# donglinb/ORB-SLAM-BIRDVIEW

Measured on AMD Instinct MI355X. Metric: ORB features/sec per GPU (1280×720, 2000 kp, 8 levels) + Hamming matches/sec, higher is better.
Workload: dtype u8; 1 GPU; C3 1280x720 KITTI-style synthetic, 2000 features, 8 levels; width=1280, height=720, nfeatures=2000, nlevels=8, ini_th_fast=20, min_th_fast=7, batch_per_gpu=256, global_batch=256, parallelism=frame-sharded x1 (no collective), batches_in_flight=2

## Files before the change

orb-slam-birdview_amd/csrc/extract_kernels.hip:

```cpp
#include "glibc_trig.h"
#include "orbgpu_internal.h"
#include "pattern31_data.inc"

#include <algorithm>
#include <cstring>

namespace orbgpu {

__constant__ __attribute__((aligned(16))) int8_t c_pattern[1024] = {ORBGPU_PATTERN31_VALUES};
__constant__ __attribute__((aligned(16))) float c_pattern_f[1024] = {ORBGPU_PATTERN31_VALUES};

struct IcMaskTable {
    uint32_t m[64][4];
};
constexpr IcMaskTable make_ic_masks() {
    IcMaskTable t{};
    constexpr int umax[16] = {15, 15, 15, 15, 14, 14, 14, 13, 13, 12, 11, 10, 9, 8, 6, 3};
    for (int l = 0; l < 64; l++) {
        const int r = (l >> 1) < 30 ? (l >> 1) : 30, v = r - 15, h = l & 1;
        const int d = umax[v < 0 ? -v : v];
        for (int i = 0; i < 4; i++) {
            uint32_t m = 0;
            for (int j = 0; j < 4; j++) {
                const int u = 4 * (4 * h + i) + j;
// ... 786 lines not shown
    for (int j = 0; j < 4; j++) {
        const uint32_t P12 = __builtin_amdgcn_alignbyte(D[j + 1], D[j], 2);
        const uint32_t P4 = __builtin_amdgcn_alignbyte(D[j + 4], D[j + 3], 2);
        r[j] = compass2(D[j + 2], P[j], P4, M[j], P12, tt);
    }
    const uint32_t X = __builtin_amdgcn_perm(r[1], r[0], 0x07050301u);
    const uint32_t Y = __builtin_amdgcn_perm(r[3], r[2], 0x07050301u);
    const uint32_t Z = ((X >> 7) & 0x01010101u) | ((Y >> 3) & 0x10101010u);
    return __builtin_amdgcn_udot4(Z, 0x08040201u, 0u, false);
}

template <int TQ, bool TAIL>
__device__ __forceinline__ int prefilter_cell(const uint32_t* t32, int dh, int rpi, int lrow, bool lane_on, int lbase,
                                              uint32_t xvalid, uint32_t tt, uint16_t* sList, const FastCellT& c,
                                              const uint16_t* tile, int lane) {
    int nlist = 0;
    const int ntail = TAIL ? __builtin_amdgcn_readfirstlane(c.ntail) : 0;
    dh -= ntail;
    for (int r0 = 0; r0 < dh; r0 += rpi) {
        const int dy = r0 + lrow;
        int pm = 0;
        if (lane_on && dy < dh) {
            lds_cu32* w = (lds_cu32*)(t32 + r0 * (TQ / 2));
            asm volatile("" : "+v"(w));
            pm = (int)((prefilter16<TQ>(w, tt) | (prefilter16<TQ>(w + 4, tt) << 8)) & xvalid);
        }
        const int cnt = __popc(pm);
        const int incl = wave_incl_scan(cnt);
        int pos = nlist + incl - cnt;
        const int base = lbase + r0 * (2 * TQ);
        for (uint32_t b = (uint32_t)pm; b; b &= b - 1) sList[pos++] = (uint16_t)(base + 2 * __builtin_ctz(b));
        nlist += __builtin_amdgcn_readlane(incl, 63);
    }
    if (TAIL && ntail != 0) {
        const int np = __builtin_amdgcn_readfirstlane(c.np);
        const int trow = (int)div20(lane, c.m_np), pp = lane - trow * np;
        uint32_t r = 0;
        if (trow < ntail) {
            lds_cu32* q = (lds_cu32*)(reinterpret_cast<const uint32_t*>(tile) + ((dh + 3) * (TQ / 2) + 2)) +
                          (trow * (TQ / 2) + pp);
            const uint32_t l2 = q[-2], l1 = q[-1], v = q[0], r1 = q[1], r2 = q[2];
            const uint32_t P12 = __builtin_amdgcn_alignbyte(l1, l2, 2);
            const uint32_t P4 = __builtin_amdgcn_alignbyte(r2, r1, 2);
            r = compass2(v, q[3 * (TQ / 2)], P4, q[-3 * (TQ / 2)], P12, tt);
        }
        const bool lo = (r & 0x8000u) != 0, hi = (int)r < 0 && 2 * pp + 1 < c.dw;
        const unsigned long long ml = __ballot(lo), mh = __ballot(hi);
        const int pos = __builtin_amdgcn_mbcnt_hi((unsigned)(mh >> 32), __builtin_amdgcn_mbcnt_lo((unsigned)mh,
                        __builtin_amdgcn_mbcnt_hi((unsigned)(ml >> 32), __builtin_amdgcn_mbcnt_lo((unsigned)ml, nlist))));
        const int e = (dh + trow) * (2 * TQ) + 4 * pp;
        if (lo) sList[pos] = (uint16_t)e;
        if (hi) sList[pos + (lo ? 1 : 0)] = (uint16_t)(e + 2);
        nlist += __popcll(ml) + __popcll(mh);
    }
    return nlist;
}

template <int TQ, int CP = 0>
__device__ __forceinline__ void fast_cell_body(const Geom* __restrict__ g, const FastCellT& c, int lane,
                                               uint16_t* tile, uint16_t* sList,
                                               uint32_t* __restrict__ cands, uint32_t* __restrict__ candFirst,
                                               int* cntOut, unsigned long long* __restrict__ stamps, int item) {
    constexpr int PX = 16, TB = 2 * TQ;
    constexpr unsigned kRecipTB = (1u << 20) / TB + 1;
    const int dw = c.dw, dh = c.dh;
    ORBGPU_STAMP(1);
    const int nruns = c.nruns;
    const int rpi = c.rpi;
    const int lrow = (int)div20(lane, c.m_runs);
    const int x0 = PX * (lane - lrow * nruns);
    const bool lane_on = lrow < rpi;
    const uint32_t xvalid = x0 + PX <= dw ? (1u << PX) - 1u : (1u << max(dw - x0, 0)) - 1u;
    const int lpix = lrow * TQ + x0;
    const uint32_t* t32 = reinterpret_cast<const uint32_t*>(tile) + (lpix >> 1);
    uint8_t* t0 = reinterpret_cast<uint8_t*>(&tile[3 * TQ + 4]);
    int th = g->iniTh;
    int kept = 0;
    for (int pass = 0; pass < 2; pass++) {
        const uint32_t tt = (uint32_t)th | ((uint32_t)th << 16);
        const int nlist = prefilter_cell<TQ, (TQ < kFastTilePitch)>(t32, dh, rpi, lrow, lane_on, 2 * lpix, xvalid, tt,
                                                                    sList, c, tile, lane);
        wave_lds_sync();
        ORBGPU_STAMP(2);
#if defined(ORBGPU_FAST_CUT) && ORBGPU_FAST_CUT == 2
        if (lane == 0) *cntOut = nlist & 0;
        return;
#endif
        int ncorner = 0;
        for (int b0 = 0; b0 < nlist; b0 += 64) {
            const int i = b0 + lane;
            int p = 0, m = 0;
            if (i < nlist) {
                p = sList[i];
                m = fast_arc_strength<TB, 2>(t0 + p);
            }
            const bool corner = m > th;
            const unsigned long long cm = __ballot(corner);
            if (corner) {
                t0[p + 1] = (uint8_t)m;
                sList[ncorner + lanes_below(cm)] = (uint16_t)p;
            }
            ncorner += __popcll(cm);
        }
        wave_lds_sync();
        ORBGPU_STAMP(3);
#if defined(ORBGPU_FAST_CUT) && ORBGPU_FAST_CUT == 3
        if (lane == 0) *cntOut = ncorner & 0;
        return;
#endif
        kept = 0;
        for (int b0 = 0; b0 < ncorner; b0 += 64) {
            const int i = b0 + lane;
            bool k = false;
            uint32_t packed = 0;
            if (i < ncorner) {
                const int p = sList[i];
                const uint8_t* q = t0 + p + 1;
                const int m = q[0];
                const int s = m - 1;
                const int n0 = max(max((int)q[-TB - 2], (int)q[-TB]), (int)q[-TB + 2]);
                const int n1 = max(max((int)q[-2], (int)q[2]), 1);
                const int n2 = max(max((int)q[TB - 2], (int)q[TB]), (int)q[TB + 2]);
                k = m > max(max(n0, n1), n2);
                const int py = (int)(__umul24((unsigned)p, kRecipTB) >> 20), px = (p - py * TB) >> 1;
                packed = (uint32_t)(px + c.xo) | ((uint32_t)(py + c.yo) << 12) | ((uint32_t)s << 24);
            }
            const unsigned long long km = __ballot(k);
            const int slot = kept + lanes_below(km);
            if (k) {
                if constexpr (CP != 0) {
                    uint32_t* dst = slot < kCandFirst ? &candFirst[((long long)c.f * g->ncells + c.cell) * kCandRec + 1 + slot]
                                                      : &cands[(long long)c.f * g->ncand + c.out_off + slot];
                    __hip_atomic_store(dst, packed, __ATOMIC_RELAXED, __HIP_MEMORY_SCOPE_AGENT);
                } else {
                    if (slot < kCandFirst) candFirst[((long long)c.f * g->ncells + c.cell) * kCandRec + 1 + slot] = packed;
                    else cands[(long long)c.f * g->ncand + c.out_off + slot] = packed;
                }
            }
            kept += __popcll(km);
        }
        if (kept > 0 || th == g->minTh) break;
        th = g->minTh;
        for (int i = lane; i < ncorner; i += 64) t0[sList[i] + 1] = 0;
        wave_lds_sync();
    }
    ORBGPU_STAMP(4);
    if (lane == 0) {
        if constexpr (CP != 0) __hip_atomic_store(cntOut, kept, __ATOMIC_RELAXED, __HIP_MEMORY_SCOPE_AGENT);
        else *cntOut = kept;
    }
    ORBGPU_STAMP(5);
}

template <int TQ>
__global__ __launch_bounds__(256) void k_fast_wave(const Geom* __restrict__ g, const CellDesc* __restrict__ cells,
                                                   const uint8_t* __restrict__ frames,
                                                   long long framePitch, int rowStride, const uint8_t* __restrict__ pyr,
                                                   uint32_t* __restrict__ cands, uint32_t* __restrict__ candFirst,
                                                   int total,
                                                   int cbeg, int cnum, unsigned long long* __restrict__ stamps,
                                                   int* __restrict__ err, int ipw) {
    extern __shared__ __attribute__((aligned(16))) int smem_fast[];
    uint8_t* smem = reinterpret_cast<uint8_t*>(smem_fast);
    const int wv = __builtin_amdgcn_readfirstlane(threadIdx.x >> 6), lane = threadIdx.x & 63;
    const int nb = gridDim.x, q = nb >> 3, r = nb & 7, xcd = blockIdx.x & 7, j = blockIdx.x >> 3;
    const int blk = (xcd < r ? xcd * (q + 1) : r * (q + 1) + (xcd - r) * q) + j;
    const int item0 = (blk * (int)(blockDim.x >> 6) + wv) * ipw;
    if (item0 >= total) return;
    const int wb = g->fast_wave_bytes;
    uint16_t* tile = reinterpret_cast<uint16_t*>(smem + (size_t)wv * wb + 16);
    uint16_t* sList = reinterpret_cast<uint16_t*>(smem + (size_t)wv * wb + ((g->fast_rows * TQ * 2 + 32 + 15) & ~15));
    const bool has1 = ipw == 2 && item0 + 1 < total;
    const FastCellT c0 = fast_cell_t(g, cells, item0, frames, framePitch, rowStride, pyr, cbeg, cnum);
    const FastCellT c1 = fast_cell_t(g, cells, has1 ? item0 + 1 : item0, frames, framePitch, rowStride, pyr, cbeg, cnum);
    u32x2_t v0[8], v1[8];
    if (c0.valid && c0.aligned) fast_roi_issue(c0, lane, v0);
    if (has1 && c1.valid && c1.aligned) fast_roi_issue(c1, lane, v1);
    if (err && blockIdx.x == 0 && threadIdx.x == 0) {
        err[0] = 0;
        if (cnum == g->ncells) err[1] = 0;
    }
#pragma unroll
    for (int k = 0; k < 2; k++) {
        if (k == 1 && !has1) break;
        const FastCellT& c = k == 0 ? c0 : c1;
        const int item = item0 + k;
        int* cntOut = reinterpret_cast<int*>(candFirst + ((long long)c.f * g->ncells + c.cell) * kCandRec);
        if (!c.valid) {
            if (lane == 0) *cntOut = 0;
            continue;
        }
        ORBGPU_STAMP(0);
        wave_lds_sync();
        fast_roi_store<TQ>(c, lane, k == 0 ? v0 : v1, tile);
        ORBGPU_STAMP(6);
#if defined(ORBGPU_FAST_CUT) && ORBGPU_FAST_CUT == 1
        wave_lds_sync();
        if (lane == 0) *cntOut = (int)tile[lane] & 0;
        continue;
#endif
        fast_cell_body<TQ>(g, c, lane, tile, sList, cands, candFirst, cntOut, stamps, item);
    }
}

void fast_wave_layout(Geom& g) {
    int rows = 1, drows = 1, list = 1, maxw = 1;
    for (int l = 0; l < g.nlevels; l++) {
        const LevelGeom& L = g.L[l];
        rows = std::max(rows, L.hCell + 6);
        drows = std::max(drows, L.hCell);
        list = std::max(list, L.hCell * L.wCell);
        maxw = std::max(maxw, L.wCell);
    }
    g.fast_rows = rows;
    g.fast_drows = drows;
    g.fast_list = list;
    g.fast_compact = maxw <= 36 ? 1 : 0;
    const int tq = g.fast_compact ? 48 : kFastTilePitch;
    g.fast_wave_bytes = ((rows * tq * 2 + 32 + 15) & ~15) + ((list * 2 + 15) & ~15);
    g.fast_wave_bytes = (g.fast_wave_bytes + 15) & ~15;
}

__device__ __forceinline__ int quadrant_of(uint32_t key, uint32_t rx, uint32_t ry) {
    const int x = key & 0xFFF, y = (key >> 12) & 0xFFF;
    const int x0 = rx & 0xFFFF, x1 = rx >> 16, y0 = ry & 0xFFFF, y1 = ry >> 16;
    const int hx = (x1 - x0 + 1) >> 1, hy = (y1 - y0 + 1) >> 1;
    return (x >= x0 + hx ? 1 : 0) | (y >= y0 + hy ? 2 : 0);
}

__device__ __forceinline__ void child_rect(uint32_t rx, uint32_t ry, int q, uint32_t& crx, uint32_t& cry) {
    const int x0 = rx & 0xFFFF, x1 = rx >> 16, y0 = ry & 0xFFFF, y1 = ry >> 16;
    const int hx = (x1 - x0 + 1) >> 1, hy = (y1 - y0 + 1) >> 1;
    const int xm = x0 + hx, ym = y0 + hy;
    const int cx0 = (q & 1) ? xm : x0, cx1 = (q & 1) ? x1 : xm;
    const int cy0 = (q & 2) ? ym : y0, cy1 = (q & 2) ? y1 : ym;
    crx = (uint32_t)cx0 | ((uint32_t)cx1 << 16);
    cry = (uint32_t)cy0 | ((uint32_t)cy1 << 16);
}

template <int CP>
__device__ __forceinline__ int tidx() {
    if constexpr (CP == 0) return threadIdx.x;
    int t;
    asm volatile("v_mov_b32 %0, %1" : "=v"(t) : "v"((int)threadIdx.x));
    return t;
}

template <int NT, int CP = 0>
__device__ __forceinline__ int oct_scan(int v, int* sc, int& par, int& total) {
    constexpr int NW = NT / 64;
    const int lane = tidx<CP>() & 63, wave = tidx<CP>() >> 6;
    const int x = wave_incl_scan(v);
    int* buf = sc + 16 * par;
    par ^= 1;
    if (lane == 63) buf[wave] = x;
    __syncthreads();
    int pre = 0, tot = 0;
#pragma unroll
    for (int i = 0; i < NW; i++) {
        const int t = buf[i];
        pre += i < wave ? t : 0;
        tot += t;
    }
    total = tot;
    return pre + x - v;
}

template <int CP = 0>
__device__ __forceinline__ void wave_agg_add(int* ctr, bool ok, int tgt) {
    unsigned long long pending = __ballot(ok);
    while (pending) {
        const int leader = __ffsll((long long)pending) - 1;
        const int tl = __builtin_amdgcn_readlane(tgt, leader);
        const unsigned long long m = __ballot(ok && tgt == tl);
        if ((int)(tidx<CP>() & 63) == leader) atomicAdd(&ctr[tl], __popcll(m));
        pending &= ~m;
    }
}

__device__ __forceinline__ int quad_mask(const int* qd) {
    return (qd[0] > 0) | ((qd[1] > 0) << 1) | ((qd[2] > 0) << 2) | ((qd[3] > 0) << 3);
}

constexpr int kFfMaxDepth = 6;
constexpr int kFfPosShift = 20;
static_assert(kFfMaxNodes <= 1 << (32 - kFfPosShift), "a list position must fit above the count");

__device__ __forceinline__ int ff_depth(int nIni, int N, int room) {
    int F = 0, tot = 0, want = kFfMaxDepth;
    for (int d = 1; d <= kFfMaxDepth; d++)
        if ((nIni << (2 * d)) >= N) {
            want = d;
            break;
        }
    for (int d = 1; d <= want && d <= kFfMaxDepth; d++) {
        const int sz = nIni << (2 * d);
        if (sz > 65536 || tot + sz > room) break;
        tot += sz;
        F = d;
    }
    return F;
}

__device__ __forceinline__ int ff_base(int nIni, int d) { return nIni * (((1 << (2 * d)) - 4) / 3); }

template <int CP, class T>
__device__ __forceinline__ void oct_out(T* p, T v) {
    if constexpr (CP != 0) __hip_atomic_store(p, v, __ATOMIC_RELAXED, __HIP_MEMORY_SCOPE_AGENT);
    else *p = v;
}

template <bool KeysInLds, int NT, int CP = 0>
__device__ __forceinline__ void octree_level(const Geom* __restrict__ g, const LevelGeom& L, int f, int l, int* smem,
                                             int C, uint32_t* keys, uint16_t* knode, uint32_t* __restrict__ lvlKps,
                                             int* __restrict__ lvlCount, int* __restrict__ err, int par,
                                             unsigned long long* __restrict__ ost) {
    const int NC = g->node_cap;
    const int tid = tidx<CP>();
    const int tieMask = (g->variant & ORB_VARIANT_TIE_REVERSE) ? 0xFFFFFF : 0;
    uint32_t* rxA = (uint32_t*)smem;
    uint32_t* ryA = rxA + NC;
    int* cntA = (int*)(ryA + NC);
    int* seqA = cntA + NC;
    uint32_t* rxB = (uint32_t*)(seqA + NC);
    uint32_t* ryB = rxB + NC;
    int* cntB = (int*)(ryB + NC);
    int* seqB = cntB + NC;
    int* quad = seqB + NC;
    int* rank = quad + 4 * NC;
    int* info = rank + NC;
    int* ord = info + NC;
    int* nchr = ord + NC;
    int* sc = nchr + NC;
    int* sv = sc + 32;
#if ORBGPU_KERNEL_STAMPS
#define OCT_STAMP(k) \
    if (ost && tid == 0) ost[(k)] = __builtin_amdgcn_s_memtime();
#else
#define OCT_STAMP(k)
#endif

    __syncthreads();
    OCT_STAMP(1);
    if (ost && tid == 0) ost[29] = (unsigned long long)C;

    const int N = L.nfeat;
    const int nIni = L.nIni;
    const float hX = L.hX;
    const int Hn = L.maxBY - kMinBorder;
    if (nIni > NC) {
        if (tid == 0) { atomicOr(err, 1); oct_out<CP>(&lvlCount[f * g->nlevels + l], 0); }
        return;
    }
    int S = 0, nextSeq = 0, phase = 1, round0 = 0;
    bool ffDone = false, quadReady = false;
    const int F = C < (1 << 20) ? ff_depth(nIni, N, 8 * NC) : 0;
    if (F > 0) {
        int* T = quad;
        int* ffc = reinterpret_cast<int*>(rxB);
        const int bF = ff_base(nIni, F);
        const int szF = nIni << (2 * F);
        for (int t = tid; t < szF; t += NT) T[bF + t] = 0;
        for (int t = tid; t < 2 * (kFfMaxDepth + 1); t += NT) ffc[t] = 0;
        __syncthreads();
        OCT_STAMP(12);
        for (int i = tid; i < C; i += NT) {
            const uint32_t k = keys[i];
            const int x = k & 0xFFF, y = (k >> 12) & 0xFFF;
            const int t = min((int)((float)x / hX), nIni - 1);
            int x0 = (int)(hX * (float)t), x1 = (int)(hX * (float)(t + 1)), y0 = 0, y1 = Hn;
            int code = t;
            for (int d = 1; d <= F; d++) {
                const int xm = x0 + ((x1 - x0 + 1) >> 1), ym = y0 + ((y1 - y0 + 1) >> 1);
                const bool bx = x >= xm, by = y >= ym;
                x0 = bx ? xm : x0;
                x1 = bx ? x1 : xm;
                y0 = by ? ym : y0;
                y1 = by ? y1 : ym;
                code = code * 4 + ((int)bx | ((int)by << 1));
            }
            knode[i] = (uint16_t)code;
            atomicAdd(&T[bF + code], 1);
        }
        __syncthreads();
        OCT_STAMP(13);
        for (int d = F - 1; d >= 0; d--) {
            const int sz = d == 0 ? nIni : nIni << (2 * d);
            int* td = d == 0 ? cntB : T + ff_base(nIni, d);
            const int* tc = T + ff_base(nIni, d + 1);
            int dn = 0, en = 0, d0 = 0, e0 = 0;
            for (int c = tid; c < sz; c += NT) {
                const int4 ch = *reinterpret_cast<const int4*>(&tc[4 * c]);
                const int pc = ch.x + ch.y + ch.z + ch.w;
                td[c] = pc;
                if (pc >= 2) {
                    dn += (ch.x > 0) + (ch.y > 0) + (ch.z > 0) + (ch.w > 0);
                    en += (ch.x > 1) + (ch.y > 1) + (ch.z > 1) + (ch.w > 1);
                }
                d0 += pc > 0;
                e0 += pc > 1;
            }
            dn = wave_sum(dn);
            en = wave_sum(en);
            if ((tidx<CP>() & 63) == 0 && (dn | en)) {
                atomicAdd(&ffc[2 * (d + 1)], dn);
                atomicAdd(&ffc[2 * (d + 1) + 1], en);
            }
            if (d == 0) {
                d0 = wave_sum(d0);
                e0 = wave_sum(e0);
                if ((tidx<CP>() & 63) == 0 && (d0 | e0)) {
                    atomicAdd(&ffc[0], d0);
                    atomicAdd(&ffc[1], e0);
                }
            }
            __syncthreads();
        }
        OCT_STAMP(14);
        int Sr = ffc[0], Eprev = ffc[1], R = 0, base = 0, nseq = 0;
        bool fin = false, ph2 = false, over = false;
        for (int r = 1; r <= F; r++) {
            const int Dr = ffc[2 * r], Er = ffc[2 * r + 1];
            const int prev = Sr;
            Sr = Sr - Eprev + Dr;
            base = nseq;
            nseq += Dr;
            R = r;
            if (Sr > NC) { over = true; break; }
            if (Sr >= N || Sr == prev) { fin = true; break; }
            if (Sr + Er * 3 > N) { ph2 = true; break; }
            Eprev = Er;
        }
        if (over) {
            if (tid == 0) { atomicOr(err, 2); oct_out<CP>(&lvlCount[f * g->nlevels + l], 0); }
            return;
        }
        const int DR = ffc[2 * R];
        int V = 0;
        for (int d = R; d >= 0; d--) V += d == 0 ? nIni : nIni << (2 * d);
        OCT_STAMP(15);
        int run = 0;
        for (int v0 = 0; v0 < V; v0 += NT) {
            const int v = v0 + tid;
            int c = 0, n = 0, d = 0;
            bool on = false;
            int* td = cntB;
            if (v < V) {
                int off = 0;
                d = R;
                for (;;) {
                    const int sz = d == 0 ? nIni : nIni << (2 * d);
                    if (v < off + sz) break;
                    off += sz;
                    d--;
                }
                const int p = v - off;
                const int lowMask = (1 << (2 * d)) - 1;
                const int rt = p >> (2 * d);
                c = (((d & 1) ? nIni - 1 - rt : rt) << (2 * d)) | ((p & lowMask) ^ (0x33333333 & lowMask));
                td = d == 0 ? cntB : T + ff_base(nIni, d);
                n = td[c] & 0xFFFFF;
                const int* ptab = d == 1 ? cntB : T + ff_base(nIni, d > 1 ? d - 1 : 1);
                const bool node = n > 0 && (d == 0 || (ptab[c >> 2] & 0xFFFFF) >= 2);
                on = node && (d == R || n == 1);
            }
            int tot;
            const int pos = run + oct_scan<NT, CP>(on ? 1 : 0, sc, par, tot);
            if (on) {
                const int t = c >> (2 * d);
                int x0 = (int)(hX * (float)t), x1 = (int)(hX * (float)(t + 1)), y0 = 0, y1 = Hn;
                for (int k2 = d - 1; k2 >= 0; k2--) {
                    const int q = (c >> (2 * k2)) & 3;
                    const int xm = x0 + ((x1 - x0 + 1) >> 1), ym = y0 + ((y1 - y0 + 1) >> 1);
                    x0 = (q & 1) ? xm : x0;
                    x1 = (q & 1) ? x1 : xm;
                    y0 = (q & 2) ? ym : y0;
                    y1 = (q & 2) ? y1 : ym;
                }
                rxA[pos] = (uint32_t)x0 | ((uint32_t)x1 << 16);
                ryA[pos] = (uint32_t)y0 | ((uint32_t)y1 << 16);
                cntA[pos] = n;
                seqA[pos] = d == 0 ? -1 - t : d == R ? base + DR - 1 - pos : base;
                td[c] = (int)((uint32_t)n | ((uint32_t)pos << kFfPosShift));
                if (d == R) ryB[pos] = (uint32_t)c;
            }
            run += tot;
        }
        __syncthreads();
        OCT_STAMP(16);
        for (int i = tid; i < C; i += NT) {
            const int code = knode[i];
            int node = 0;
            for (int d = 0; d <= R; d++) {
                const int c = code >> (2 * (F - d));
                const int e = d == 0 ? cntB[c] : T[ff_base(nIni, d) + c];
                if (d == R || (e & 0xFFFFF) == 1) {
                    node = (int)((uint32_t)e >> kFfPosShift);
                    break;
                }
            }
            knode[i] = (uint16_t)node;
        }
        if (ph2 && R + 1 <= F) {
            constexpr int kMaxPer = 8;
            static_assert(kMaxPer * NT >= kFfMaxNodes, "every node of the list is read by some thread");
            int4 qv[kMaxPer];
            const int* tq = T + ff_base(nIni, R + 1);
#pragma unroll
            for (int j = 0; j < kMaxPer; j++) {
                const int pos = tid + j * NT;
                qv[j] = make_int4(0, 0, 0, 0);
                if (pos < run && pos < DR && cntA[pos] >= 2) qv[j] = *reinterpret_cast<const int4*>(&tq[4 * (int)ryB[pos]]);
            }
            __syncthreads();
#pragma unroll
            for (int j = 0; j < kMaxPer; j++) {
                const int pos = tid + j * NT;
                if (pos < run) *reinterpret_cast<int4*>(&quad[4 * pos]) = qv[j];
            }
            quadReady = true;
        }
        S = run;
        nextSeq = nseq;
        round0 = R;
        ffDone = fin;
        if (ph2) phase = 2;
    } else {
        for (int t = tid; t < nIni; t += NT) cntB[t] = 0;
        __syncthreads();
        for (int i0 = 0; i0 < C; i0 += NT) {
            const int i = i0 + tid;
            const bool ok = i < C;
            int r = 0;
            if (ok) {
                const int x = keys[i] & 0xFFF;
                r = min((int)((float)x / hX), nIni - 1);
                knode[i] = (uint16_t)r;
            }
            wave_agg_add<CP>(cntB, ok, r);
        }
        __syncthreads();
        for (int t0 = 0; t0 < nIni; t0 += NT) {
            const int t = t0 + tid;
            const int n = t < nIni ? cntB[t] : 0;
            int tot;
            const int pos = S + oct_scan<NT, CP>(n > 0 ? 1 : 0, sc, par, tot);
            if (n > 0) {
                const int x0 = (int)(hX * (float)t), x1 = (int)(hX * (float)(t + 1));
                rxA[pos] = (uint32_t)x0 | ((uint32_t)x1 << 16);
                ryA[pos] = (uint32_t)Hn << 16;
                cntA[pos] = n;
                seqA[pos] = -1 - t;
            }
            if (t < nIni) info[t] = pos;
            S += tot;
        }
        __syncthreads();
        for (int i = tid; i < C; i += NT) knode[i] = (uint16_t)info[knode[i]];
    }
    if (tid == 0) sv[3] = 0;
    __syncthreads();
    OCT_STAMP(2);

    for (int round = round0; round < 4 * NC + 64 && !ffDone; round++) {
        const int prevSize = S;
        [[maybe_unused]] const int subBase = round == 0 ? 12 : phase == 2 ? 20 : -1;
#if ORBGPU_KERNEL_STAMPS
#define OCT_SUB(k) \
    if (ost && tid == 0 && subBase >= 0 && subBase + (k) < 29) ost[subBase + (k)] = __builtin_amdgcn_s_memtime();
#else
#define OCT_SUB(k)
#endif
        if (!quadReady) for (int t = tid; t < 4 * S; t += NT) quad[t] = 0;
        for (int t = tid; t < S; t += NT) rank[t] = -1;
        __syncthreads();
        OCT_SUB(0);
        for (int i0 = 0; i0 < (quadReady ? 0 : C); i0 += 4 * NT) {
            int tt[4], tg[4];
            uint32_t kk[4];
            bool inc[4];
#pragma unroll
            for (int u = 0; u < 4; u++) {
                const int ic = min(i0 + u * NT + tid, C - 1);
                tt[u] = knode[ic];
                kk[u] = keys[ic];
            }
#pragma unroll
            for (int u = 0; u < 4; u++) {
                const int t = tt[u];
                inc[u] = i0 + u * NT + tid < C && cntA[t] > 1;
                tg[u] = 4 * t + quadrant_of(kk[u], rxA[t], ryA[t]);
            }
#pragma unroll
            for (int u = 0; u < 4; u++)
                if (inc[u]) atomicAdd(&quad[tg[u]], 1);
        }
        if (tid == 0) sv[4] = 0;
        __syncthreads();
        OCT_SUB(1);
        quadReady = false;
        int CH = 0, ndiv = 0;
        if (phase == 1) {
            int nproc = 0;
            for (int t0 = 0; t0 < S; t0 += NT) {
                const int t = t0 + tid;
                int val = 0, mask = 0;
                if (t < S && cntA[t] > 1) {
                    mask = quad_mask(&quad[4 * t]);
                    val = 1 | (__popc(mask) << 16);
                }
                int tot;
                const int pre = oct_scan<NT, CP>(val, sc, par, tot);
                if (t < S) {
                    if (val) {
                        rank[t] = nproc + (pre & 0xFFFF);
                        nchr[t] = CH + (pre >> 16);
                        info[t] = mask << 16;
                    } else {
                        info[t] = t - nproc - (pre & 0xFFFF);
                    }
                }
                nproc += tot & 0xFFFF;
                CH += tot >> 16;
            }
            ndiv = nproc;
            OCT_SUB(2);
        } else {
            int* dd = cntB;
            int* dpre = seqB;
            int nsort = 0;
            constexpr int kRkV = 32, NWv = NT / 64;
            const bool binned = 2 * NC >= kRkV * 16 && NC >= kRkV;
            if (binned) {
                int* T2 = reinterpret_cast<int*>(rxB);
                int* HV = seqB;
                int* ovl = nchr;
                const int lane = tid & 63, wave = tid >> 6;
                const bool rev = tieMask != 0;
                if (lane < kRkV) T2[lane * 16 + wave] = 0;
                const int PW = (S + NWv - 1) / NWv;
                const unsigned long long below = (1ull << lane) - 1ull;
                for (int c0 = wave * PW; c0 < min(S, (wave + 1) * PW); c0 += 64) {
                    const int pidx = c0 + lane;
                    const bool in = pidx < min(S, (wave + 1) * PW);
                    const int t = rev ? S - 1 - pidx : pidx;
                    const int cnt = in ? cntA[t] : 0;
                    const bool bg = cnt > 1;
                    const int v = min(cnt, kRkV - 1);
                    unsigned long long m = __ballot(bg);
#pragma unroll
                    for (int b = 0; b < 5; b++) {
                        const unsigned long long bal = __ballot((v >> b) & 1);
                        m &= ((v >> b) & 1) ? bal : ~bal;
                    }
                    const int prev = bg ? T2[v * 16 + wave] : 0;
                    __builtin_amdgcn_wave_barrier();
                    if (bg && (m & below) == 0) T2[v * 16 + wave] = prev + __popcll(m);
                    wave_lds_sync();
                    if (bg) {
                        info[t] = prev + __popcll(m & below);
                        if (v == kRkV - 1) ovl[atomicAdd(&sv[4], 1)] = t;
                    }
                }
                __syncthreads();
                for (int i = tid; i < kRkV * 16; i += NT) {
                    const int x = (i & 15) < NWv ? T2[i] : 0;
                    int y = x;
                    y += __builtin_amdgcn_update_dpp(0, y, 0x111, 0xf, 0xf, true);
                    y += __builtin_amdgcn_update_dpp(0, y, 0x112, 0xf, 0xf, true);
                    y += __builtin_amdgcn_update_dpp(0, y, 0x114, 0xf, 0xf, true);
                    y += __builtin_amdgcn_update_dpp(0, y, 0x118, 0xf, 0xf, true);
                    T2[i] = y - x;
                    if ((i & 15) == 15) HV[i >> 4] = y;
                }
                __syncthreads();
#pragma unroll 1
                for (int i = 0; i < kRkV; i += 4) {
                    const int4 h = *reinterpret_cast<const int4*>(&HV[i]);
                    nsort += h.x + h.y + h.z + h.w;
                }
                const int nov = sv[4];
                for (int t = tid; t < S; t += NT) {
                    const int cnt = cntA[t];
                    if (cnt <= 1) continue;
                    const int v = min(cnt, kRkV - 1);
                    const int pidx = rev ? S - 1 - t : t;
                    int r = 0;
                    if (v < kRkV - 1) {
                        r = info[t] + T2[v * 16 + pidx / PW];
#pragma unroll 1
                        for (int i = (v + 1) & ~3; i < kRkV; i += 4) {
                            const int4 h = *reinterpret_cast<const int4*>(&HV[i]);
                            r += (i > v ? h.x : 0) + (i + 1 > v ? h.y : 0) + (i + 2 > v ? h.z : 0) + (i + 3 > v ? h.w : 0);
                        }
                    } else {
                        for (int i = 0; i < nov; i++) {
                            const int u = ovl[i];
                            const int cu = cntA[u], pu = rev ? S - 1 - u : u;
                            r += cu > cnt || (cu == cnt && pu < pidx);
                        }
                    }
                    ord[r] = t;
                    dd[r] = __popc(quad_mask(&quad[4 * t])) - 1;
                }
                if (tid == 0) sv[2] = nsort;
                OCT_SUB(2);
            } else {
                unsigned long long* skey = reinterpret_cast<unsigned long long*>(rxB);
                for (int t0 = 0; t0 < S; t0 += NT) {
                    const int t = t0 + tid;
                    const bool big = t < S && cntA[t] > 1;
                    int tot;
                    const int pos = nsort + oct_scan<NT, CP>(big ? 1 : 0, sc, par, tot);
                    if (big)
                        skey[pos] = ((unsigned long long)cntA[t] << 40) |
                                    ((unsigned long long)((unsigned)(seqA[t] ^ tieMask) & 0xFFFFFFu) << 16) |
                                    (unsigned long long)t;
                    nsort += tot;
                }
                if (tid == 0) sv[2] = nsort;
                __syncthreads();
                OCT_SUB(2);
                const int G = nsort <= NT / 8 ? 8 : nsort <= NT / 4 ? 4 : nsort <= NT / 2 ? 2 : 1;
                const int lg = tid & (G - 1);
                for (int j0 = 0; j0 < nsort * G; j0 += NT) {
                    const int j = (j0 + tid) / G;
                    const bool ok = j < nsort;
                    const unsigned long long key = ok ? skey[j] : ~0ull;
                    int r = 0;
                    for (int i = 8 * lg; i + 8 <= nsort; i += 8 * G) {
                        const ulonglong2* p = reinterpret_cast<const ulonglong2*>(skey + i);
                        const ulonglong2 a = p[0], b = p[1], c = p[2], d = p[3];
                        r += (a.x > key) + (a.y > key) + (b.x > key) + (b.y > key) + (c.x > key) + (c.y > key) +
                             (d.x > key) + (d.y > key);
                    }
                    if (lg == 0)
                        for (int i = nsort & ~7; i < nsort; i++) r += skey[i] > key;
                    for (int o = 1; o < G; o <<= 1) r += __shfl_xor(r, o);
                    if (ok && lg == 0) {
                        const int t = (int)(key & 0xFFFF);
                        ord[r] = t;
                        dd[r] = __popc(quad_mask(&quad[4 * t])) - 1;
                    }
                }
            }
            __syncthreads();
            OCT_SUB(3);
            int run = 0;
            for (int r0 = 0; r0 < nsort; r0 += NT) {
                const int r = r0 + tid;
                const int d = r < nsort ? dd[r] : 0;
                int tot;
                const int pre = run + oct_scan<NT, CP>(d, sc, par, tot);
                if (r < nsort) dpre[r] = pre;
                const unsigned long long fail = __ballot(r < nsort && S + pre + d >= N);
                if (fail && (tidx<CP>() & 63) == 0) atomicMin(&sv[2], r0 + (tid & ~63) + __ffsll((long long)fail) - 1);
                run += tot;
            }
            __syncthreads();
            OCT_SUB(4);
            const int first_stop = sv[2];
            const int nproc = first_stop < nsort ? first_stop + 1 : nsort;
            ndiv = nproc;
            CH = nproc > 0 ? dpre[nproc - 1] + dd[nproc - 1] + nproc : 0;
            for (int r = tid; r < nproc; r += NT) {
                const int t = ord[r];
                rank[t] = r;
                nchr[t] = dpre[r] + r;
                info[t] = quad_mask(&quad[4 * t]) << 16;
            }
            __syncthreads();
            OCT_SUB(5);
            int und = 0;
            for (int t0 = 0; t0 < S; t0 += NT) {
                const int t = t0 + tid;
                const bool keep = t < S && rank[t] < 0;
                int tot;
                const int pre = und + oct_scan<NT, CP>(keep ? 1 : 0, sc, par, tot);
                if (keep) info[t] = pre;
                und += tot;
            }
            OCT_SUB(6);
        }
        const int Snew = CH + S - ndiv;
        if (Snew > NC) {
            if (tid == 0) { atomicOr(err, 2); oct_out<CP>(&lvlCount[f * g->nlevels + l], 0); }
            return;
        }
        int big = 0;
        for (int t0 = 0; t0 < S; t0 += NT) {
            const int t = t0 + tid;
            if (t >= S) break;
            const int rk = rank[t], inf = info[t], P = nchr[t], cnt = cntA[t], sq = seqA[t];
            const uint32_t rx = rxA[t], ry = ryA[t];
            const int4 qd = *reinterpret_cast<const int4*>(&quad[4 * t]);
            if (rk >= 0) {
                const int qc[4] = {qd.x, qd.y, qd.z, qd.w};
                const int mask = inf >> 16;
                const int start = CH - P - __popc(mask);
#pragma unroll
                for (int q = 0; q < 4; q++) {
                    if (!(mask & (1 << q))) continue;
                    const int pos = start + __popc(mask >> (q + 1));
                    uint32_t crx, cry;
                    child_rect(rx, ry, q, crx, cry);
                    rxB[pos] = crx;
                    ryB[pos] = cry;
                    cntB[pos] = qc[q];
                    seqB[pos] = nextSeq + P + __popc(mask & ((1 << q) - 1));
                    big += qc[q] > 1;
                }
                info[t] = start | (mask << 16);
            } else {
                const int pos = CH + inf;
                rxB[pos] = rx;
                ryB[pos] = ry;
                cntB[pos] = cnt;
                seqB[pos] = sq;
                info[t] = pos;
            }
        }
        big = wave_sum(big);
        if ((tidx<CP>() & 63) == 0 && big) atomicAdd(&sv[3], big);
        __syncthreads();
        OCT_SUB(phase == 1 ? 3 : 7);
        for (int i0 = 0; i0 < C; i0 += 4 * NT) {
            int tt[4], nt[4];
            uint32_t kk[4];
#pragma unroll
            for (int u = 0; u < 4; u++) {
                const int ic = min(i0 + u * NT + tid, C - 1);
                tt[u] = knode[ic];
                kk[u] = keys[ic];
            }
#pragma unroll
            for (int u = 0; u < 4; u++) {
                const int t = tt[u];
                const int inf = info[t], rk = rank[t];
                const int q = quadrant_of(kk[u], rxA[t], ryA[t]);
                nt[u] = rk >= 0 ? (inf & 0xFFFF) + __popc((inf >> 16) >> (q + 1)) : inf;
            }
#pragma unroll
            for (int u = 0; u < 4; u++)
                if (i0 + u * NT + tid < C) knode[i0 + u * NT + tid] = (uint16_t)nt[u];
        }
        const int nToExpand = sv[3];
        __syncthreads();
        OCT_SUB(phase == 1 ? 4 : 8);
        if (tid == 0) sv[3] = 0;
        {
            uint32_t* p = rxA; rxA = rxB; rxB = p;
            p = ryA; ryA = ryB; ryB = p;
            int* q = cntA; cntA = cntB; cntB = q;
            q = seqA; seqA = seqB; seqB = q;
        }
        nextSeq += CH;
        S = Snew;
        if (round < 9) OCT_STAMP(3 + round);
        if (S >= N || S == prevSize) break;
        if (phase == 1 && S + nToExpand * 3 > N) {
            phase = 2;
            if (ost && tid == 0) ost[30] = (unsigned long long)(round + 1);
        }
    }

#undef OCT_SUB
    uint32_t* best = (uint32_t*)quad;
    for (int t = tid; t < S; t += NT) best[t] = 0;
    __syncthreads();
    OCT_STAMP(17);
    for (int i = tid; i < C; i += NT) {
        const uint32_t v = ((keys[i] >> 24) << 24) | (uint32_t)(0xFFFFFF - i);
        atomicMax(&best[knode[i]], v);
    }
    __syncthreads();
    OCT_STAMP(18);
    uint32_t* outK = lvlKps + (long long)f * g->nkpcap + L.kp_base;
    for (int t = tid; t < S; t += NT) {
        const int i = 0xFFFFFF - (int)(best[t] & 0xFFFFFF);
        const uint32_t k = keys[i];
        const uint32_t x = (k & 0xFFF) + kMinBorder, y = ((k >> 12) & 0xFFF) + kMinBorder;
        oct_out<CP>(&outK[t], x | (y << 12) | (k & 0xFF000000u));
    }
    if (tid == 0) oct_out<CP>(&lvlCount[f * g->nlevels + l], S);
    OCT_STAMP(31);
#undef OCT_STAMP
}

template <int CP>
__device__ __forceinline__ uint32_t cand_slot(__amdgpu_buffer_rsrc_t rs, unsigned i) {
    return __builtin_amdgcn_raw_buffer_load_b32(rs, (int)(4 * i), 0, CP);
}

template <int NT, int CP>
__device__ __forceinline__ void octree_task(const Geom* __restrict__ g, int f, int l, int* smem,
                                            const uint32_t* __restrict__ cands, const uint32_t* __restrict__ candFirst,
                                            uint32_t* __restrict__ keysAll, uint16_t* __restrict__ knodeAll,
                                            uint32_t* __restrict__ lvlKps, int* __restrict__ lvlCount,
                                            int* __restrict__ err, int lds_keys, unsigned long long* __restrict__ ostamps) {
    const int NC = g->node_cap;
    const int tid = tidx<CP>();
    const LevelGeom& L = g->L[l];
    unsigned long long* ost = ostamps ? ostamps + ((long long)f * g->nlevels + l) * 32 : nullptr;
#if ORBGPU_KERNEL_STAMPS
    if (ost && tid == 0) ost[0] = __builtin_amdgcn_s_memtime();
#endif
    constexpr int kFirst = kCandFirst;
    const int ncl = L.nCols * L.nRows;
    const uint32_t* cs = cands + (long long)f * g->ncand + L.cand_base;
    const uint4* cf = reinterpret_cast<const uint4*>(candFirst) + ((long long)f * g->ncells + L.cell_base) * 2;
    const uint32_t* cr = candFirst + ((long long)f * g->ncells + L.cell_base) * kCandRec;
    static_assert(kCandRec == 8, "two uint4 per cell record");
    auto crsf = [&]() { return __builtin_amdgcn_make_buffer_rsrc(const_cast<uint32_t*>(cr), 0, ncl * kCandRec * 4, 0x00020000); };
    auto csrf = [&]() { return __builtin_amdgcn_make_buffer_rsrc(const_cast<uint32_t*>(cs), 0, L.cand_cap * 4, 0x00020000); };
    int* sc = smem + 16 * NC;
    int* sv = sc + 32;
    uint32_t* keysL = reinterpret_cast<uint32_t*>(sv + 8);
    const long long o = ((long long)f * g->nlevels + l) * g->max_level_cand;
    int par = 0;
    constexpr int kMaxChunks = 4;
    const int nch = (ncl + NT - 1) / NT;
    int C = 0;
    bool inLds;
    uint32_t* keys;
    if (nch <= kMaxChunks) {
        int n[kMaxChunks], off[kMaxChunks];
        uint32_t v[kMaxChunks][kFirst];
#pragma unroll
        for (int j = 0; j < kMaxChunks; j++) {
            n[j] = 0;
#pragma unroll
            for (int k = 0; k < kFirst; k++) v[j][k] = 0;
            const int c = j * NT + tid;
            if (j < nch && c < ncl) {
                uint4 r0, r1;
                if constexpr (CP != 0) {
                    const uint32x4_t a = __builtin_amdgcn_raw_buffer_load_b128(crsf(), 32 * c, 0, CP);
                    const uint32x4_t b = __builtin_amdgcn_raw_buffer_load_b128(crsf(), 32 * c + 16, 0, CP);
                    r0 = make_uint4(a[0], a[1], a[2], a[3]);
                    r1 = make_uint4(b[0], b[1], b[2], b[3]);
                } else {
                    r0 = cf[2 * c];
                    r1 = cf[2 * c + 1];
                }
                n[j] = (int)r0.x;
                v[j][0] = r0.y;
                v[j][1] = r0.z;
                v[j][2] = r0.w;
                v[j][3] = r1.x;
                v[j][4] = r1.y;
                v[j][5] = r1.z;
                v[j][6] = r1.w;
            }
        }
#pragma unroll
        for (int j = 0; j < kMaxChunks; j++) {
            if (j < nch) {
                int tot;
                off[j] = C + oct_scan<NT, CP>(n[j], sc, par, tot);
                C += tot;
            }
        }
        inLds = C <= lds_keys;
        keys = inLds ? keysL : keysAll + o;
#pragma unroll
        for (int j = 0; j < kMaxChunks; j++) {
            const int c = j * NT + tid;
            if (j < nch && c < ncl) {
#pragma unroll
                for (int k = 0; k < kFirst; k++)
                    if (k < n[j]) keys[off[j] + k] = v[j][k];
                if constexpr (CP != 0) {
                    for (int k = kFirst; k < n[j]; k++) keys[off[j] + k] = cand_slot<CP>(csrf(), __umul24((unsigned)c, (unsigned)L.cell_cap) + k);
                } else {
                    for (int k = kFirst; k < n[j]; k++) keys[off[j] + k] = cs[__umul24((unsigned)c, (unsigned)L.cell_cap) + k];
                }
            }
        }
    } else {
        int base = 0;
        for (int c0 = 0; c0 < ncl; c0 += NT) {
            const int c = c0 + tid;
            int n = 0;
            if constexpr (CP != 0) n = c < ncl ? (int)cand_slot<CP>(crsf(), (unsigned)c * kCandRec) : 0;
            else n = c < ncl ? (int)cr[(long long)c * kCandRec] : 0;
            int tot;
            (void)oct_scan<NT, CP>(n, sc, par, tot);
            base += tot;
        }
        C = base;
        inLds = C <= lds_keys;
        keys = inLds ? keysL : keysAll + o;
        base = 0;
        for (int c0 = 0; c0 < ncl; c0 += NT) {
            const int c = c0 + tid;
            int n = 0;
            if constexpr (CP != 0) n = c < ncl ? (int)cand_slot<CP>(crsf(), (unsigned)c * kCandRec) : 0;
            else n = c < ncl ? (int)cr[(long long)c * kCandRec] : 0;
            int tot;
            const int off = base + oct_scan<NT, CP>(n, sc, par, tot);
            if constexpr (CP != 0) {
                for (int k = 0; k < n; k++)
                    keys[off + k] = k < kFirst ? cand_slot<CP>(crsf(), (unsigned)c * kCandRec + 1 + k)
                                               : cand_slot<CP>(csrf(), __umul24((unsigned)c, (unsigned)L.cell_cap) + k);
            } else {
                for (int k = 0; k < n; k++)
                    keys[off + k] = k < kFirst ? cr[(long long)c * kCandRec + 1 + k]
                                               : cs[__umul24((unsigned)c, (unsigned)L.cell_cap) + k];
            }
            base += tot;
        }
    }
    if (inLds)
        octree_level<true, NT, CP>(g, L, f, l, smem, C, keys, reinterpret_cast<uint16_t*>(keysL + lds_keys), lvlKps, lvlCount,
                               err, par, ost);
    else
        octree_level<false, NT, CP>(g, L, f, l, smem, C, keys, knodeAll + o, lvlKps, lvlCount, err, par, ost);
}


template <int NT>
__global__ __launch_bounds__(NT) void k_octree(const Geom* __restrict__ g,
                                                           const uint32_t* __restrict__ cands,
                                                           const uint32_t* __restrict__ candFirst,
                                                           uint32_t* __restrict__ keysAll,
                                                           uint16_t* __restrict__ knodeAll,
                                                           uint32_t* __restrict__ lvlKps, int* __restrict__ lvlCount,
                                                           int* __restrict__ err, int lds_keys,
                                                           unsigned long long* __restrict__ ostamps, int lbase) {
    extern __shared__ __attribute__((aligned(16))) int smem[];
    octree_task<NT, 0>(g, blockIdx.x, lbase + (int)blockIdx.y, smem, cands, candFirst, keysAll, knodeAll, lvlKps,
                       lvlCount, err, lds_keys, ostamps);
}

constexpr float kAtanScale = (float)(180 / 3.14159265358979323846);
constexpr float kP1 = 0.9997878412794807f * kAtanScale;
constexpr float kP3 = -0.3258083974640975f * kAtanScale;
constexpr float kP5 = 0.1555786518463281f * kAtanScale;
constexpr float kP7 = -0.04432655554792128f * kAtanScale;
constexpr float kFactorPI = (float)(3.14159265358979323846 / 180.f);

__device__ __forceinline__ float fast_atan2(float y, float x) {
    const float ax = fabsf(x), ay = fabsf(y);
    float a, c, c2;
    if (ax >= ay) {
        c = ay / (ax + (float)2.220446049250313e-16);
        c2 = c * c;
        a = (((kP7 * c2 + kP5) * c2 + kP3) * c2 + kP1) * c;
    } else {
        c = ax / (ay + (float)2.220446049250313e-16);
        c2 = c * c;
        a = 90.f - (((kP7 * c2 + kP5) * c2 + kP3) * c2 + kP1) * c;
    }
    if (x < 0) a = 180.f - a;
    if (y < 0) a = 360.f - a;
    return a;
}



constexpr int kDescRtCols = 37, kDescWinOff = 2976, kDescWaveBytes = kDescWinOff + kDescWin * kDescWinPitch;
constexpr bool desc_overlap_ok() {
    return 2 * kRtPitch * kDescRtCols <= kDescWinOff + 6 * kDescWinPitch && kDescWinOff % 16 == 0 &&
           kDescWaveBytes % 16 == 0 && 4 * kDescWaveBytes + 256 <= 160 * 1024 / 8;
}
static_assert(desc_overlap_ok(), "k_describe LDS overlap");

struct DescSlot {
    bool ok, interior;
    int s, l, x, y, score, outIdx;
    LevelPtr src;
};

template <int CP = 0>
__device__ __forceinline__ DescSlot desc_slot(const Geom* __restrict__ g, int f, int s, const int* cnts,
                                              const uint32_t* __restrict__ lvlKps, const uint8_t* frames,
                                              long long framePitch, int rowStride, const uint8_t* pyr) {
    DescSlot d;
    d.s = s;
    d.ok = false;
    d.interior = false;
    if (s >= g->nkpcap) return d;
    const int nl = g->nlevels;
    int l = 0;
    while (l + 1 < nl && s >= g->L[l + 1].kp_base) ++l;
    const LevelGeom& L = g->L[l];
    const int k = s - L.kp_base;
    auto cnt = [&](int i) -> int {
        if constexpr (CP != 0) return __hip_atomic_load(&cnts[i], __ATOMIC_RELAXED, __HIP_MEMORY_SCOPE_AGENT);
        else return cnts[i];
    };
    if (k >= cnt(l)) return d;
    int outIdx = k;
    for (int i = 0; i < l; i++) outIdx += cnt(i);
    uint32_t kp;
    if constexpr (CP != 0) kp = __hip_atomic_load(&lvlKps[(long long)f * g->nkpcap + s], __ATOMIC_RELAXED, __HIP_MEMORY_SCOPE_AGENT);
    else kp = lvlKps[(long long)f * g->nkpcap + s];
    d.ok = true;
    d.l = l;
    d.x = kp & 0xFFF;
    d.y = (kp >> 12) & 0xFFF;
    d.score = kp >> 24;
    d.outIdx = outIdx;
    d.src = level_ptr(g, l, frames, framePitch, rowStride, pyr, f);
    const bool aligned = ((reinterpret_cast<uintptr_t>(d.src.p) | (uintptr_t)d.src.stride) & 3) == 0;
    d.interior = aligned && d.x >= 21 && d.x + 27 <= L.w && d.y >= 21 && d.y + 21 < L.h;
    return d;
}

template <int CP = 0>
__device__ __forceinline__ void desc_issue(const DescSlot& d, int lane, uint32_t (&v)[9]) {
    const int a0 = (d.x - 21) & ~3;
    const int stride = __builtin_amdgcn_readfirstlane(d.src.stride);
    const uint64_t rb = reinterpret_cast<uint64_t>(d.src.p + (long long)(d.y - 21) * stride + a0);
    const uint64_t rbu = ((uint64_t)(uint32_t)__builtin_amdgcn_readfirstlane((unsigned)(rb >> 32)) << 32) |
                         (uint64_t)(uint32_t)__builtin_amdgcn_readfirstlane((unsigned)rb);
    const auto rsrc = __builtin_amdgcn_make_buffer_rsrc(reinterpret_cast<void*>(rbu), 0, (kDescWin - 1) * stride + 48,
                                                          0x00020000);
    const int wy0 = (int)(__umul24((unsigned)lane, 2731u) >> 15), ww = lane - wy0 * 12;
    const int off = (int)roi_off(wy0, stride, 4 * ww);
#pragma unroll
    for (int r = 0; r < 8; r++) v[r] = __builtin_amdgcn_raw_buffer_load_b32(rsrc, off, 5 * r * stride, CP);
    v[8] = __builtin_amdgcn_raw_buffer_load_b32(rsrc, lane < 36 ? off : 0x40000000, 40 * stride, CP);
}

template <bool ALLEVEN, bool FMA>
__device__ __forceinline__ void brief_sampled(const uint16_t* rt, float a, float b, const float (&pf)[4][4], int colBase,
                                              int xsimd, ushort2_t K01, ushort2_t K23, ushort2_t K45, ushort2_t K60,
                                              int lane, unsigned long long* __restrict__ dst) {
    typedef const uint32_t __attribute__((address_space(3))) lds_u32;
    constexpr uint32_t kC = (uint32_t)kRtPitch * 0x400000u + 0x4B400000u;
    static_assert((kC & 1u) == 0, "the element bias must keep the parity");
    const uint32_t lbase = (uint32_t)(uintptr_t)(lds_u32*)reinterpret_cast<const uint32_t*>(rt) - 2u * kC;
    const uint32_t xlim = (uint32_t)(xsimd - colBase) + 0x4B400000u;
    const uint32_t bias = sgpr_const(32767u);
    typedef float f32x2_t __attribute__((ext_vector_type(2)));
    const f32x2_t ab = {a, b}, nba = {-b, a}, cr = {12582930.0f, 12582930.0f};
    auto sample = [&](f32x2_t pp) -> uint32_t {
        const f32x2_t pyv = __builtin_shufflevector(pp, pp, 1, 1), pxv = __builtin_shufflevector(pp, pp, 0, 0);
        const f32x2_t t = pyv * nba;
        const f32x2_t r = (FMA ? __builtin_elementwise_fma(pxv, ab, t) : pxv * ab + t) + cr;
        const float fx = r.x, fy = r.y;
        const uint32_t xbits = __builtin_bit_cast(uint32_t, fx);
        const uint32_t ybits = __builtin_bit_cast(uint32_t, fy);
        const uint32_t idx = __umul24(xbits, (unsigned)kRtPitch) + ybits;
        uint32_t ie = idx & ~1u;
        asm("" : "+v"(ie));
        lds_u32* rp = (lds_u32*)(uintptr_t)(lbase + (ie << 1));
        const uint32_t sh = idx << 4;
        const uint32_t d0 = rp[0], d1 = rp[1], d2 = rp[2], d3 = rp[3];
        uint32_t S = __builtin_amdgcn_udot2(K01, __builtin_bit_cast(ushort2_t, __builtin_amdgcn_alignbit(d1, d0, sh)), 0u, false);
        S = __builtin_amdgcn_udot2(K23, __builtin_bit_cast(ushort2_t, __builtin_amdgcn_alignbit(d2, d1, sh)), S, false);
        S = __builtin_amdgcn_udot2(K45, __builtin_bit_cast(ushort2_t, __builtin_amdgcn_alignbit(d3, d2, sh)), S, false);
        S = __builtin_amdgcn_udot2(K60, __builtin_bit_cast(ushort2_t, __builtin_amdgcn_alignbit(d3, d3, sh)), S, false);
        if (ALLEVEN) return S + bias + ((S >> 16) & 1u);
        return S + (xbits < xlim ? bias + ((S >> 16) & 1u) : 32768u);
    };
    unsigned long long mq[4];
#pragma unroll
    for (int gq = 0; gq < 4; gq++) {
        const uint32_t r0 = sample(f32x2_t{pf[gq][0], pf[gq][1]});
        const uint32_t r1 = sample(f32x2_t{pf[gq][2], pf[gq][3]});
        mq[gq] = __ballot((r0 >> 16) < min(r1 >> 16, 255u));
    }
    if (lane < 4) dst[lane] = lane == 0 ? mq[0] : lane == 1 ? mq[1] : lane == 2 ? mq[2] : mq[3];
}

// ... 890 lines not shown
```

Baseline: 410.4 million features/s.

## Drive phase-2 octree rounds from precomputed fast-forward count tables

Builds the fast-forward quadtree count table one level deeper and, when phase 2 begins within that depth, represents nodes as packed (depth, code) pairs. Child counts are then read directly from the table instead of rebucketing every keypoint each round. Keypoint-to-node assignment is deferred to a single lookup pass at the end, or runs when the tree grows past the tabled depth, at which point rectangles are reconstructed. The goal is to remove the per-round passes over all keypoints in the octree distribution. In exchange it uses more shared-memory table space, adds extra code paths, and adds a final fixup pass.

```diff
diff --git a/orb-slam-birdview_amd/csrc/extract_kernels.hip b/orb-slam-birdview_amd/csrc/extract_kernels.hip
--- a/orb-slam-birdview_amd/csrc/extract_kernels.hip
+++ b/orb-slam-birdview_amd/csrc/extract_kernels.hip
@@ -1112,7 +1112,28 @@
     return F;
 }
 
+__device__ __forceinline__ uint32_t ff_pack(int d, int c) { return ((uint32_t)d << 16) | (uint32_t)c; }
+
+__device__ __forceinline__ void ff_rect(float hX, int Hn, int d, int c, uint32_t& rx, uint32_t& ry) {
+    const int t = c >> (2 * d);
+    int x0 = (int)(hX * (float)t), x1 = (int)(hX * (float)(t + 1)), y0 = 0, y1 = Hn;
+    for (int k2 = d - 1; k2 >= 0; k2--) {
+        const int q = (c >> (2 * k2)) & 3;
+        const int xm = x0 + ((x1 - x0 + 1) >> 1), ym = y0 + ((y1 - y0 + 1) >> 1);
+        x0 = (q & 1) ? xm : x0;
+        x1 = (q & 1) ? x1 : xm;
+        y0 = (q & 2) ? ym : y0;
+        y1 = (q & 2) ? y1 : ym;
+    }
+    rx = (uint32_t)x0 | ((uint32_t)x1 << 16);
+    ry = (uint32_t)y0 | ((uint32_t)y1 << 16);
+}
+
 __device__ __forceinline__ int ff_base(int nIni, int d) { return nIni * (((1 << (2 * d)) - 4) / 3); }
+
+__device__ __forceinline__ int ff_table_depth(int nIni, int F, int keep) {
+    return F > 0 && (nIni << (2 * (F + 1))) <= 65536 && ff_base(nIni, F + 2) <= keep ? F + 1 : F;
+}
 
 template <int CP, class T>
 __device__ __forceinline__ void oct_out(T* p, T v) {
@@ -1164,14 +1185,17 @@
     }
     int S = 0, nextSeq = 0, phase = 1, round0 = 0;
     bool ffDone = false, quadReady = false;
+    bool tabled = false;
+    int Dp = 0;
     const int F = C < (1 << 20) ? ff_depth(nIni, N, 8 * NC) : 0;
+    const int D = ff_table_depth(nIni, F, 4 * NC);
     if (F > 0) {
         int* T = quad;
         int* ffc = reinterpret_cast<int*>(rxB);
-        const int bF = ff_base(nIni, F);
-        const int szF = nIni << (2 * F);
+        const int bF = ff_base(nIni, D);
+        const int szF = nIni << (2 * D);
         for (int t = tid; t < szF; t += NT) T[bF + t] = 0;
-        for (int t = tid; t < 2 * (kFfMaxDepth + 1); t += NT) ffc[t] = 0;
+        for (int t = tid; t < 2 * (kFfMaxDepth + 2); t += NT) ffc[t] = 0;
         __syncthreads();
         OCT_STAMP(12);
         for (int i = tid; i < C; i += NT) {
@@ -1180,7 +1204,7 @@
             const int t = min((int)((float)x / hX), nIni - 1);
             int x0 = (int)(hX * (float)t), x1 = (int)(hX * (float)(t + 1)), y0 = 0, y1 = Hn;
             int code = t;
-            for (int d = 1; d <= F; d++) {
+            for (int d = 1; d <= D; d++) {
                 const int xm = x0 + ((x1 - x0 + 1) >> 1), ym = y0 + ((y1 - y0 + 1) >> 1);
                 const bool bx = x >= xm, by = y >= ym;
                 x0 = bx ? xm : x0;
@@ -1194,7 +1218,7 @@
         }
         __syncthreads();
         OCT_STAMP(13);
-        for (int d = F - 1; d >= 0; d--) {
+        for (int d = D - 1; d >= 0; d--) {
             const int sz = d == 0 ? nIni : nIni << (2 * d);
             int* td = d == 0 ? cntB : T + ff_base(nIni, d);
             const int* tc = T + ff_base(nIni, d + 1);
@@ -1246,6 +1270,9 @@
             return;
         }
         const int DR = ffc[2 * R];
+        for (int d = 1; d <= D; d++)
+            if (ff_base(nIni, d + 1) <= 4 * NC) Dp = d;
+        tabled = ph2 && R + 1 <= Dp;
         int V = 0;
         for (int d = R; d >= 0; d--) V += d == 0 ? nIni : nIni << (2 * d);
         OCT_STAMP(15);
@@ -1278,31 +1305,28 @@
             const int pos = run + oct_scan<NT, CP>(on ? 1 : 0, sc, par, tot);
             if (on) {
                 const int t = c >> (2 * d);
-                int x0 = (int)(hX * (float)t), x1 = (int)(hX * (float)(t + 1)), y0 = 0, y1 = Hn;
-                for (int k2 = d - 1; k2 >= 0; k2--) {
-                    const int q = (c >> (2 * k2)) & 3;
-                    const int xm = x0 + ((x1 - x0 + 1) >> 1), ym = y0 + ((y1 - y0 + 1) >> 1);
-                    x0 = (q & 1) ? xm : x0;
-                    x1 = (q & 1) ? x1 : xm;
-                    y0 = (q & 2) ? ym : y0;
-                    y1 = (q & 2) ? y1 : ym;
+                if (tabled) {
+                    ryA[pos] = ff_pack(d, c);
+                } else {
+                    uint32_t rx, ry;
+                    ff_rect(hX, Hn, d, c, rx, ry);
+                    rxA[pos] = rx;
+                    ryA[pos] = ry;
                 }
-                rxA[pos] = (uint32_t)x0 | ((uint32_t)x1 << 16);
-                ryA[pos] = (uint32_t)y0 | ((uint32_t)y1 << 16);
                 cntA[pos] = n;
                 seqA[pos] = d == 0 ? -1 - t : d == R ? base + DR - 1 - pos : base;
                 td[c] = (int)((uint32_t)n | ((uint32_t)pos << kFfPosShift));
-                if (d == R) ryB[pos] = (uint32_t)c;
+                if (d == R && !tabled) ryB[pos] = (uint32_t)c;
             }
             run += tot;
         }
         __syncthreads();
         OCT_STAMP(16);
-        for (int i = tid; i < C; i += NT) {
+        for (int i = tid; i < (tabled ? 0 : C); i += NT) {
             const int code = knode[i];
             int node = 0;
             for (int d = 0; d <= R; d++) {
-                const int c = code >> (2 * (F - d));
+                const int c = code >> (2 * (D - d));
                 const int e = d == 0 ? cntB[c] : T[ff_base(nIni, d) + c];
                 if (d == R || (e & 0xFFFFF) == 1) {
                     node = (int)((uint32_t)e >> kFfPosShift);
@@ -1311,7 +1335,7 @@
             }
             knode[i] = (uint16_t)node;
         }
-        if (ph2 && R + 1 <= F) {
+        if (ph2 && R + 1 <= F && !tabled) {
             constexpr int kMaxPer = 8;
             static_assert(kMaxPer * NT >= kFfMaxNodes, "every node of the list is read by some thread");
             int4 qv[kMaxPer];
@@ -1368,9 +1392,43 @@
         __syncthreads();
         for (int i = tid; i < C; i += NT) knode[i] = (uint16_t)info[knode[i]];
     }
-    if (tid == 0) sv[3] = 0;
+    if (tid == 0) sv[3] = sv[5] = 0;
     __syncthreads();
     OCT_STAMP(2);
+    auto quad_of = [&](int t) -> int4 {
+        if (!tabled) return *reinterpret_cast<const int4*>(&quad[4 * t]);
+        const uint32_t dc = ryA[t];
+        const int4 e = *reinterpret_cast<const int4*>(&quad[ff_base(nIni, (int)(dc >> 16) + 1) + 4 * (int)(dc & 0xFFFF)]);
+        return make_int4(e.x & 0xFFFFF, e.y & 0xFFFFF, e.z & 0xFFFFF, e.w & 0xFFFFF);
+    };
+    auto mask_of = [&](int t) -> int {
+        const int4 q = quad_of(t);
+        return (q.x > 0) | ((q.y > 0) << 1) | ((q.z > 0) << 2) | ((q.w > 0) << 3);
+    };
+    auto keys_to_nodes = [&]() {
+        for (int t = tid; t < S; t += NT) {
+            const uint32_t dc = ryA[t];
+            const int d = (int)(dc >> 16), c = (int)(dc & 0xFFFF);
+            if (d == 0) rank[c] = t;
+            else quad[ff_base(nIni, d) + c] = (int)((uint32_t)cntA[t] | ((uint32_t)t << kFfPosShift));
+        }
+        __syncthreads();
+        for (int i = tid; i < C; i += NT) {
+            const int code = knode[i];
+            int node = -1;
+            for (int d = Dp; d >= 1; d--) {
+                const int c = code >> (2 * (D - d));
+                const int p = (int)((uint32_t)quad[ff_base(nIni, d) + c] >> kFfPosShift);
+                if (ryA[p] == ff_pack(d, c)) {
+                    node = p;
+                    break;
+                }
+            }
+            if (node < 0) node = rank[code >> (2 * D)];
+            knode[i] = (uint16_t)node;
+        }
+        __syncthreads();
+    };
 
     for (int round = round0; round < 4 * NC + 64 && !ffDone; round++) {
         const int prevSize = S;
@@ -1381,11 +1439,11 @@
 #else
 #define OCT_SUB(k)
 #endif
-        if (!quadReady) for (int t = tid; t < 4 * S; t += NT) quad[t] = 0;
+        if (!quadReady && !tabled) for (int t = tid; t < 4 * S; t += NT) quad[t] = 0;
         for (int t = tid; t < S; t += NT) rank[t] = -1;
         __syncthreads();
         OCT_SUB(0);
-        for (int i0 = 0; i0 < (quadReady ? 0 : C); i0 += 4 * NT) {
+        for (int i0 = 0; i0 < (quadReady || tabled ? 0 : C); i0 += 4 * NT) {
             int tt[4], tg[4];
             uint32_t kk[4];
             bool inc[4];
@@ -1511,7 +1569,7 @@
                         }
                     }
                     ord[r] = t;
-                    dd[r] = __popc(quad_mask(&quad[4 * t])) - 1;
+                    dd[r] = __popc(mask_of(t)) - 1;
                 }
                 if (tid == 0) sv[2] = nsort;
                 OCT_SUB(2);
@@ -1550,7 +1608,7 @@
                     if (ok && lg == 0) {
                         const int t = (int)(key & 0xFFFF);
                         ord[r] = t;
-                        dd[r] = __popc(quad_mask(&quad[4 * t])) - 1;
+                        dd[r] = __popc(mask_of(t)) - 1;
                     }
                 }
             }
@@ -1577,7 +1635,7 @@
                 const int t = ord[r];
                 rank[t] = r;
                 nchr[t] = dpre[r] + r;
-                info[t] = quad_mask(&quad[4 * t]) << 16;
+                info[t] = mask_of(t) << 16;
             }
             __syncthreads();
             OCT_SUB(5);
@@ -1597,13 +1655,13 @@
             if (tid == 0) { atomicOr(err, 2); oct_out<CP>(&lvlCount[f * g->nlevels + l], 0); }
             return;
         }
-        int big = 0;
+        int big = 0, deep = 0;
         for (int t0 = 0; t0 < S; t0 += NT) {
             const int t = t0 + tid;
             if (t >= S) break;
             const int rk = rank[t], inf = info[t], P = nchr[t], cnt = cntA[t], sq = seqA[t];
             const uint32_t rx = rxA[t], ry = ryA[t];
-            const int4 qd = *reinterpret_cast<const int4*>(&quad[4 * t]);
+            const int4 qd = rk >= 0 || !tabled ? quad_of(t) : make_int4(0, 0, 0, 0);
             if (rk >= 0) {
                 const int qc[4] = {qd.x, qd.y, qd.z, qd.w};
                 const int mask = inf >> 16;
@@ -1612,10 +1670,16 @@
                 for (int q = 0; q < 4; q++) {
                     if (!(mask & (1 << q))) continue;
                     const int pos = start + __popc(mask >> (q + 1));
-                    uint32_t crx, cry;
-                    child_rect(rx, ry, q, crx, cry);
-                    rxB[pos] = crx;
-                    ryB[pos] = cry;
+                    if (tabled) {
+                        const int cd = (int)(ry >> 16) + 1;
+                        ryB[pos] = ff_pack(cd, 4 * (int)(ry & 0xFFFF) + q);
+                        deep |= qc[q] > 1 && cd >= Dp;
+                    } else {
+                        uint32_t crx, cry;
+                        child_rect(rx, ry, q, crx, cry);
+                        rxB[pos] = crx;
+                        ryB[pos] = cry;
+                    }
                     cntB[pos] = qc[q];
                     seqB[pos] = nextSeq + P + __popc(mask & ((1 << q) - 1));
                     big += qc[q] > 1;
@@ -1632,9 +1696,10 @@
         }
         big = wave_sum(big);
         if ((tidx<CP>() & 63) == 0 && big) atomicAdd(&sv[3], big);
+        if (deep) sv[5] = 1;
         __syncthreads();
         OCT_SUB(phase == 1 ? 3 : 7);
-        for (int i0 = 0; i0 < C; i0 += 4 * NT) {
+        for (int i0 = 0; i0 < (tabled ? 0 : C); i0 += 4 * NT) {
             int tt[4], nt[4];
             uint32_t kk[4];
 #pragma unroll
@@ -1655,6 +1720,7 @@
                 if (i0 + u * NT + tid < C) knode[i0 + u * NT + tid] = (uint16_t)nt[u];
         }
         const int nToExpand = sv[3];
+        const bool leave = tabled && sv[5] != 0;
         __syncthreads();
         OCT_SUB(phase == 1 ? 4 : 8);
         if (tid == 0) sv[3] = 0;
@@ -1672,7 +1738,20 @@
             phase = 2;
             if (ost && tid == 0) ost[30] = (unsigned long long)(round + 1);
         }
-    }
+        if (leave) {
+            keys_to_nodes();
+            for (int t = tid; t < S; t += NT) {
+                const uint32_t dc = ryA[t];
+                uint32_t rx, ry;
+                ff_rect(hX, Hn, (int)(dc >> 16), (int)(dc & 0xFFFF), rx, ry);
+                rxA[t] = rx;
+                ryA[t] = ry;
+            }
+            tabled = false;
+            __syncthreads();
+        }
+    }
+    if (tabled) keys_to_nodes();
 
 #undef OCT_SUB
     uint32_t* best = (uint32_t*)quad;
```

Measured after the change: 404.1 million features/s. -1.5%, worse.
